# Borda/pyImSegm

Hardware: NVIDIA H100
Metric: megapixels/sec end-to-end SLIC+features+GC (pipe_color2d_slic_features_model_graphcut) (higher is better)
Workload: dtype f64

## Files before the change

### pyimsegm_b200/csrc/graph.cu

```cuda
#include "common.cuh"
#include "block_scan.cuh"
#include <cooperative_groups.h>
namespace cg = cooperative_groups;

namespace {


struct AdjWs {
    unsigned long long* table;
    int* deg;
    int* off;
    int* fill;
    int* tmp_a;
    int* ctr;
    int slots;
};

__device__ __forceinline__ unsigned hash64(unsigned long long k)
{
    k ^= k >> 33; k *= 0xff51afd7ed558ccdull; k ^= k >> 33; k *= 0xc4ceb9fe1a85ec53ull; k ^= k >> 33;
    return (unsigned)k;
}

__device__ void edge_insert(const AdjWs& w, int l0, int l1)
{
    int a = min(l0, l1), b = max(l0, l1);
    unsigned long long key = ((unsigned long long)(unsigned)b << 32) | (unsigned)a;
    unsigned mask = (unsigned)w.slots - 1u;
    unsigned h = hash64(key) & mask;
    for (int probe = 0; probe < w.slots; ++probe) {
        unsigned long long cur = w.table[h];
        if (cur == key) return;
        if (cur == ~0ull) {
            unsigned long long old = atomicCAS(&w.table[h], ~0ull, key);
            if (old == ~0ull) { atomicAdd(&w.deg[b], 1); atomicAdd(&w.ctr[0], 1); return; }
            if (old == key) return;
        }
        h = (h + 1) & mask;
    }
    atomicExch(&w.ctr[1], 1);
}

__global__ void __launch_bounds__(256) k_edge_scan(const int* __restrict__ seg, int H, int W, AdjWs w)
{
    size_t p = (size_t)blockIdx.x * blockDim.x + threadIdx.x;
    if (p >= (size_t)H * W) return;
    int y = (int)(p / W), x = (int)(p % W);
    int l = seg[p];
    if (x + 1 < W) {
        int r = seg[p + 1];
        if (r != l && !(y > 0 && seg[p - W] == l && seg[p - W + 1] == r)) edge_insert(w, l, r);
    }
    if (y + 1 < H) {
        int d = seg[p + W];
        if (d != l && !(x > 0 && seg[p - 1] == l && seg[p + W - 1] == d)) edge_insert(w, l, d);
    }
}

__global__ void __launch_bounds__(256) k_edge_scan3d(const int* __restrict__ seg, int D, int H, int W, AdjWs w)
{
    size_t p = (size_t)blockIdx.x * blockDim.x + threadIdx.x;
    if (p >= (size_t)D * H * W) return;
    const int x = (int)(p % W), y = (int)((p / W) % H), z = (int)(p / ((size_t)H * W));
    const int l = seg[p];
    if (x + 1 < W) { const int r = seg[p + 1]; if (r != l) edge_insert(w, l, r); }
    if (y + 1 < H) { const int d = seg[p + W]; if (d != l) edge_insert(w, l, d); }
    if (z + 1 < D) { const int b = seg[p + (size_t)H * W]; if (b != l) edge_insert(w, l, b); }
}

__global__ void k_centroid3d_acc(const int* __restrict__ seg, int D, int H, int W, unsigned long long* acc)
{
    size_t p = (size_t)blockIdx.x * blockDim.x + threadIdx.x;
    if (p >= (size_t)D * H * W) return;
    const int x = (int)(p % W), y = (int)((p / W) % H), z = (int)(p / ((size_t)H * W));
    unsigned long long* a = acc + 4 * (size_t)seg[p];
    atomicAdd(a, 1ull); atomicAdd(a + 1, (unsigned long long)z); atomicAdd(a + 2, (unsigned long long)y); atomicAdd(a + 3, (unsigned long long)x);
}

__global__ void k_centroid3d_fin(int nb, const unsigned long long* acc, double* centres)
{
    const int k = blockIdx.x * blockDim.x + threadIdx.x;
    if (k >= nb) return;
    const double c = (double)acc[4 * (size_t)k];
    for (int d = 0; d < 3; ++d) centres[3 * (size_t)k + d] = c > 0 ? (double)acc[4 * (size_t)k + 1 + d] / c : -1.0;
}

__global__ void __launch_bounds__(1024) k_edge_offsets(int nb, AdjWs w, int cap, int* n_edges_out)
{
    const int total = cta_scan_chunks<1024, int>(nb, [&](int i) { return w.deg[i]; },
                                                 [&](int i, int off) { w.off[i] = off; w.fill[i] = 0; });
    if (threadIdx.x == 0) {
        w.off[nb] = total;
        *n_edges_out = (w.ctr[1] || total > cap) ? cap + 1 : total;
    }
}

__global__ void k_edge_fill(AdjWs w, int cap)
{
    int i = blockIdx.x * blockDim.x + threadIdx.x;
    if (i >= w.slots) return;
    unsigned long long key = w.table[i];
    if (key == ~0ull) return;
    int b = (int)(key >> 32), a = (int)(key & 0xffffffffu);
    int pos = w.off[b] + atomicAdd(&w.fill[b], 1);
    if (pos < cap) w.tmp_a[pos] = a;
}

__global__ void k_edge_emit(int nb, AdjWs w, int cap, int* __restrict__ edges)
{
    int b = blockIdx.x * blockDim.x + threadIdx.x;
    if (b >= nb) return;
    int beg = w.off[b], end = w.off[b + 1];
    if (end > cap) return;
    for (int i = beg + 1; i < end; ++i) {
        int v = w.tmp_a[i], j = i - 1;
        while (j >= beg && w.tmp_a[j] > v) { w.tmp_a[j + 1] = w.tmp_a[j]; --j; }
        w.tmp_a[j + 1] = v;
    }
    for (int i = beg; i < end; ++i) { edges[2 * (size_t)i] = w.tmp_a[i]; edges[2 * (size_t)i + 1] = b; }
}

static int pow2_at_least(long long v) { int p = 1024; while (p < v) p <<= 1; return p; }

static size_t carve_adj(AdjWs& w, void* ws, size_t bytes, int nb, int cap)
{
    WsCarver c(ws, bytes);
    w.slots = pow2_at_least(2LL * cap);
    w.table = c.take<unsigned long long>((size_t)w.slots);
    w.deg = c.take<int>(nb);
    w.off = c.take<int>((size_t)nb + 1);
    w.fill = c.take<int>(nb);
    w.tmp_a = c.take<int>(cap);
    w.ctr = c.take<int>(4);
    return isb_align(c.off);
}


__device__ double block_sum(double v, double* s_red)
{
#pragma unroll
    for (int o = 16; o > 0; o >>= 1) v += __shfl_xor_sync(0xffffffffu, v, o);
    __syncthreads();
    if ((threadIdx.x & 31) == 0) s_red[threadIdx.x >> 5] = v;
    __syncthreads();
    double t = 0;
    for (int i = 0; i < (int)(blockDim.x >> 5); ++i) t += s_red[i];
    return t;
}

__device__ double block_max(double v, double* s_red)
{
#pragma unroll
    for (int o = 16; o > 0; o >>= 1) v = fmax(v, __shfl_xor_sync(0xffffffffu, v, o));
    __syncthreads();
    if ((threadIdx.x & 31) == 0) s_red[threadIdx.x >> 5] = v;
    __syncthreads();
    double t = s_red[0];
    for (int i = 1; i < (int)(blockDim.x >> 5); ++i) t = fmax(t, s_red[i]);
    return t;
}

constexpr int ECL = 8;

__device__ double cluster_reduce(double v, bool is_max, double* s_red, double* s_x)
{
    const double t = is_max ? block_max(v, s_red) : block_sum(v, s_red);
    cg::cluster_group cl = cg::this_cluster();
    if (threadIdx.x == 0) *s_x = t;
    cl.sync();
    double tot = is_max ? -1.0 : 0.0;
    for (int r = 0; r < ECL; ++r) { const double pr = *cl.map_shared_rank(s_x, r); tot = is_max ? fmax(tot, pr) : tot + pr; }
    cl.sync();
    return tot;
}

__global__ void __cluster_dims__(ECL, 1, 1) __launch_bounds__(1024) k_gc_energies(const double* __restrict__ proba, int N_in, const int* n_nodes_dev, int K, const int* __restrict__ edges, int E_in,
                                                      const int* n_edges_dev, const double* __restrict__ centres,
                                                      const double* __restrict__ vfeat, int D, int metric, int spatial,
                                                      double edge_cost, const double* __restrict__ pairwise, double* unary,
                                                      double* edge_w, int* unary_i, int* edge_wi, int* smooth_i, double* sp)
{
    __shared__ double s_red[32];
    __shared__ double s_x;
    const int tid = blockIdx.x * blockDim.x + threadIdx.x, nth = gridDim.x * blockDim.x;
    const int E = n_edges_dev ? (*n_edges_dev > E_in ? 0 : *n_edges_dev) : E_in;
    const int N = n_nodes_dev ? min(*n_nodes_dev, N_in) : N_in;
    double umax = 0.0;
    for (int i = tid; i < N * K; i += nth) {
        double p = proba[i];
        if (p < 0.01) p = 0.01;
        if (p > 1.0 - 0.01) p = 1.0 - 0.01;
        double u = fabs(-log(p));
        unary[i] = u;
        umax = fmax(umax, fabs(u));
    }
    umax = cluster_reduce(umax, true, s_red, &s_x);
    double dsum = 0.0, ssum = 0.0;
    for (int e = tid; e < E; e += nth) {
        int a = edges[2 * e], b = edges[2 * e + 1];
        double dist = 0.0;
        if (metric != 0) {
            const double* va = vfeat + (size_t)a * D;
            const double* vb = vfeat + (size_t)b * D;
            for (int k = 0; k < D; ++k) {
                double df = va[k] - vb[k];
                if (metric == 1) dist = fmax(dist, df * df);
                else if (metric == 2) dist += fabs(df);
                else dist += df * df;
            }
            if (metric == 3) dist = sqrt(dist);
        }
        edge_w[e] = dist;
        dsum += dist;
        if (spatial) {
            double cy = centres[2 * a] - centres[2 * b], cx = centres[2 * a + 1] - centres[2 * b + 1];
            double s = sqrt(cy * cy + cx * cx);
            sp[e] = s;
            ssum += s;
        }
    }
    dsum = cluster_reduce(dsum, false, s_red, &s_x);
    ssum = cluster_reduce(ssum, false, s_red, &s_x);
    const double dmean = E > 0 ? dsum / E : 0.0, smean = E > 0 ? ssum / E : 1.0;
    double vsum = 0.0;
    if (metric != 0)
        for (int e = tid; e < E; e += nth) { double t = edge_w[e] - dmean; vsum += t * t; }
    vsum = cluster_reduce(vsum, false, s_red, &s_x);
    const double sd = sqrt(E > 0 ? vsum / E : 0.0);
    const double denom = 2.0 * (sd * sd);
    double wmax = 0.0;
    for (int e = tid; e < E; e += nth) {
        double wv = metric != 0 ? exp(-edge_w[e] / denom) : 1.0;
        if (spatial) wv = wv / (sp[e] / smean);
        if (wv < 1e-3) wv = 1e-3;
        if (wv > 1e3) wv = 1e3;
        wv *= edge_cost;
        edge_w[e] = wv;
        wmax = fmax(wmax, fabs(wv));
    }
    wmax = cluster_reduce(wmax, true, s_red, &s_x);
    double pmax = pairwise[0];
    for (int i = 1; i < K * K; ++i) pmax = fmax(pmax, pairwise[i]);
    const double dwf = fmax(umax, wmax * pmax) + 1e-10;
    for (int i = tid; i < N * K; i += nth) unary_i[i] = (int)((unary[i] / dwf) * 100000.0);
    for (int e = tid; e < E; e += nth) { const double wv = edge_w[e]; edge_wi[e] = isnan(wv) ? 0 : (int)((wv / dwf) * 1000.0); }
    for (int i = tid; i < K * K; i += nth) smooth_i[i] = (int)(pairwise[i] * 100.0);
}


__global__ void __launch_bounds__(256) k_gather(const int* __restrict__ seg, long long n, const int* __restrict__ lut_i,
                                                const double* __restrict__ lut_p, int K, int* __restrict__ out_i, double* __restrict__ out_p)
{
    long long p = (long long)blockIdx.x * blockDim.x + threadIdx.x;
    if (p >= n) return;
    int l = seg[p];
    if (out_i) out_i[p] = lut_i[l];
    if (out_p) {
        const double* src = lut_p + (size_t)l * K;
        double* dst = out_p + (size_t)p * K;
        for (int k = 0; k < K; ++k) dst[k] = src[k];
    }
}

}

extern "C" size_t isb_adjacency_workspace_bytes(int nb, int cap)
{
    AdjWs w;
    return carve_adj(w, nullptr, 0, nb, cap);
}

extern "C" int isb_adjacency_edges(const int32_t* seg, int H, int W, int nb, int32_t* edges, int cap, int32_t* n_edges_out, void* ws,
                                   size_t ws_bytes, isb_stream_t stream)
{
    ISB_REQUIRE(seg && edges && n_edges_out && ws, "null pointer");
    ISB_REQUIRE(H > 0 && W > 0 && nb > 0 && cap > 0, "bad sizes");
    AdjWs w;
    size_t need = carve_adj(w, ws, ws_bytes, nb, cap);
    ISB_REQUIRE(need <= ws_bytes, "workspace too small");
    cudaStream_t st = (cudaStream_t)stream;
    ProfScope prof(ISB_PROF_ADJ, st);
    ISB_CUDA_CHECK(cudaMemsetAsync(w.table, 0xFF, sizeof(unsigned long long) * (size_t)w.slots, st));
    ISB_CUDA_CHECK(cudaMemsetAsync(w.deg, 0, sizeof(int) * (size_t)nb, st));
    ISB_CUDA_CHECK(cudaMemsetAsync(w.ctr, 0, sizeof(int) * 4, st));
    size_t n = (size_t)H * W;
    k_edge_scan<<<(unsigned)((n + 255) / 256), 256, 0, st>>>(seg, H, W, w);
    ISB_LAUNCH_CHECK();
    k_edge_offsets<<<1, 1024, 0, st>>>(nb, w, cap, n_edges_out);
    ISB_LAUNCH_CHECK();
    k_edge_fill<<<(w.slots + 255) / 256, 256, 0, st>>>(w, cap);
    ISB_LAUNCH_CHECK();
    k_edge_emit<<<(nb + 127) / 128, 128, 0, st>>>(nb, w, cap, edges);
    ISB_LAUNCH_CHECK();
    return ISB_OK;
}

extern "C" int isb_adjacency_edges_3d(const int32_t* seg, int D, int H, int W, int nb, int32_t* edges, int cap, int32_t* n_edges_out,
                                      void* ws, size_t ws_bytes, isb_stream_t stream)
{
    ISB_REQUIRE(seg && edges && n_edges_out && ws, "null pointer");
    ISB_REQUIRE(D > 0 && H > 0 && W > 0 && nb > 0 && cap > 0, "bad sizes");
    AdjWs w;
    size_t need = carve_adj(w, ws, ws_bytes, nb, cap);
    ISB_REQUIRE(need <= ws_bytes, "workspace too small");
    cudaStream_t st = (cudaStream_t)stream;
    ProfScope prof(ISB_PROF_ADJ, st);
    ISB_CUDA_CHECK(cudaMemsetAsync(w.table, 0xFF, sizeof(unsigned long long) * (size_t)w.slots, st));
    ISB_CUDA_CHECK(cudaMemsetAsync(w.deg, 0, sizeof(int) * (size_t)nb, st));
    ISB_CUDA_CHECK(cudaMemsetAsync(w.ctr, 0, sizeof(int) * 4, st));
    size_t n = (size_t)D * H * W;
    k_edge_scan3d<<<(unsigned)((n + 255) / 256), 256, 0, st>>>(seg, D, H, W, w);
    ISB_LAUNCH_CHECK();
    k_edge_offsets<<<1, 1024, 0, st>>>(nb, w, cap, n_edges_out);
    ISB_LAUNCH_CHECK();
    k_edge_fill<<<(w.slots + 255) / 256, 256, 0, st>>>(w, cap);
    ISB_LAUNCH_CHECK();
    k_edge_emit<<<(nb + 127) / 128, 128, 0, st>>>(nb, w, cap, edges);
    ISB_LAUNCH_CHECK();
    return ISB_OK;
}

extern "C" int isb_centroids_3d(const int32_t* seg, int D, int H, int W, int nb, double* centres, void* ws, size_t ws_bytes, isb_stream_t stream)
{
    ISB_REQUIRE(seg && centres && ws, "null pointer");
    ISB_REQUIRE(D > 0 && H > 0 && W > 0 && nb > 0, "bad sizes");
    ISB_REQUIRE(ws_bytes >= sizeof(unsigned long long) * 4 * (size_t)nb, "workspace too small (4 * nb uint64)");
    cudaStream_t st = (cudaStream_t)stream;
    ISB_CUDA_CHECK(cudaMemsetAsync(ws, 0, sizeof(unsigned long long) * 4 * (size_t)nb, st));
    size_t n = (size_t)D * H * W;
    k_centroid3d_acc<<<(unsigned)((n + 255) / 256), 256, 0, st>>>(seg, D, H, W, (unsigned long long*)ws);
    ISB_LAUNCH_CHECK();
    k_centroid3d_fin<<<(nb + 255) / 256, 256, 0, st>>>(nb, (const unsigned long long*)ws, centres);
    ISB_LAUNCH_CHECK();
    return ISB_OK;
}

extern "C" size_t isb_gc_energies_workspace_bytes(int N, int K, int E) { return isb_align(sizeof(double) * (size_t)(E > 0 ? E : 1)); }

extern "C" int isb_gc_energies(const double* proba, int N, const int32_t* n_nodes_dev, int K, const int32_t* edges, int E, const int32_t* n_edges_dev,
                               const double* centres, int metric, int spatial, double edge_cost, const double* pairwise, double* unary,
                               double* edge_w, int32_t* unary_i, int32_t* edge_wi, int32_t* smooth_i, void* ws, size_t ws_bytes,
                               isb_stream_t stream)
{
    ISB_REQUIRE(proba && edges && pairwise && unary && edge_w && unary_i && edge_wi && smooth_i && ws, "null pointer");
    ISB_REQUIRE(N > 0 && K > 0 && E >= 0, "bad sizes");
    ISB_REQUIRE(metric >= 0 && metric <= 3, "metric must be 0..3");
    ISB_REQUIRE(!spatial || centres, "centres are required for spatially normalised edge weights");
    ISB_REQUIRE(ws_bytes >= isb_gc_energies_workspace_bytes(N, K, E), "workspace too small");
    ProfScope prof(ISB_PROF_ENERGY, (cudaStream_t)stream);
    k_gc_energies<<<ECL, 1024, 0, (cudaStream_t)stream>>>(proba, N, n_nodes_dev, K, edges, E, n_edges_dev, centres, proba, K, metric, spatial, edge_cost,
                                                         pairwise, unary, edge_w, unary_i, edge_wi, smooth_i, (double*)ws);
    ISB_LAUNCH_CHECK();
    return ISB_OK;
}

__global__ void k_fill_i32(int* p, long long n, int v)
{
    long long i = (long long)blockIdx.x * blockDim.x + threadIdx.x;
    if (i < n) p[i] = v;
}

extern "C" int isb_fill_i32(int32_t* dst, long long n, int32_t value, isb_stream_t stream)
{
    ISB_REQUIRE(dst && n > 0, "bad arguments");
    k_fill_i32<<<(unsigned)((n + 255) / 256), 256, 0, (cudaStream_t)stream>>>(dst, n, value);
    ISB_LAUNCH_CHECK();
    return ISB_OK;
}

__global__ void k_combine(void* dst, const void* src, long long n, int op)
{
    long long i = (long long)blockIdx.x * blockDim.x + threadIdx.x;
    if (i >= n) return;
    if (op == 0) ((long long*)dst)[i] += ((const long long*)src)[i];
    else if (op == 1) { long long a = ((long long*)dst)[i], b = ((const long long*)src)[i]; ((long long*)dst)[i] = a > b ? a : b; }
    else if (op == 2) ((double*)dst)[i] = fmin(((double*)dst)[i], ((const double*)src)[i]);
    else if (op == 3) ((double*)dst)[i] = fmax(((double*)dst)[i], ((const double*)src)[i]);
    else ((double*)dst)[i] = ((double*)dst)[i] + ((const double*)src)[i];
}

extern "C" int isb_combine(void* dst, const void* src, long long n, int op, isb_stream_t stream)
{
    ISB_REQUIRE(dst && src && n > 0 && op >= 0 && op <= 4, "bad arguments");
    k_combine<<<(unsigned)((n + 255) / 256), 256, 0, (cudaStream_t)stream>>>(dst, src, n, op);
    ISB_LAUNCH_CHECK();
    return ISB_OK;
}

extern "C" int isb_gather(const int32_t* seg, long long npx, const int32_t* lut_i, const double* lut_p, int K, int32_t* out_i,
                          double* out_p, isb_stream_t stream)
{
    ISB_REQUIRE(seg && npx > 0, "bad arguments");
    ISB_REQUIRE((!out_i || lut_i) && (!out_p || (lut_p && K > 0)), "LUT missing for a requested output");
    ProfScope prof(ISB_PROF_GATHER, (cudaStream_t)stream);
    k_gather<<<(unsigned)((npx + 255) / 256), 256, 0, (cudaStream_t)stream>>>(seg, npx, lut_i, lut_p, K, out_i, out_p);
    ISB_LAUNCH_CHECK();
    return ISB_OK;
}
```

### pyimsegm_b200/csrc/segment_stats.cu

```cuda
#include "common.cuh"

namespace {

constexpr int SROWS = 16;

struct StatWs {
    double* acc;
    double* var;
    long long* iacc;
    float* meanf;
};

__device__ __forceinline__ float clean(float v) { return isnan(v) ? 0.0f : v; }

__global__ void __launch_bounds__(256) k_stats_pass1(const void* __restrict__ img, int dtype, const int* __restrict__ seg, int H, int W,
                                                     int y_off, StatWs ws)
{
    const int x = blockIdx.x * 256 + threadIdx.x;
    if (x >= W) return;
    const int y0 = blockIdx.y * SROWS, y1 = min(y0 + SROWS, H);
    int cur = -1;
    double s0 = 0, s1 = 0, s2 = 0, e0 = 0, e1 = 0, e2 = 0;
    long long cnt = 0, sy = 0;
    for (int y = y0; y <= y1; ++y) {
        int l = -1;
        float v0 = 0, v1 = 0, v2 = 0;
        if (y < y1) {
            size_t p = (size_t)y * W + x;
            l = seg[p];
            if (img) {
                v0 = clean(load_as_f32(img, dtype, 3 * p));
                v1 = clean(load_as_f32(img, dtype, 3 * p + 1));
                v2 = clean(load_as_f32(img, dtype, 3 * p + 2));
            }
        }
        if (l != cur) {
            if (cur >= 0) {
                double* a = ws.acc + 6 * (size_t)cur;
                atomicAdd(a, s0); atomicAdd(a + 1, s1); atomicAdd(a + 2, s2);
                atomicAdd(a + 3, e0); atomicAdd(a + 4, e1); atomicAdd(a + 5, e2);
                unsigned long long* ia = (unsigned long long*)(ws.iacc + 3 * (size_t)cur);
                atomicAdd(ia, (unsigned long long)cnt);
                atomicAdd(ia + 1, (unsigned long long)sy);
                atomicAdd(ia + 2, (unsigned long long)(cnt * x));
            }
            cur = l;
            s0 = s1 = s2 = e0 = e1 = e2 = 0;
            cnt = 0; sy = 0;
        }
        if (y < y1) {
            s0 += (double)v0; s1 += (double)v1; s2 += (double)v2;
            e0 += (double)__fmul_rn(v0, v0); e1 += (double)__fmul_rn(v1, v1); e2 += (double)__fmul_rn(v2, v2);
            cnt += 1; sy += y + y_off;
        }
    }
}

__global__ void k_stats_means(int nb, StatWs ws)
{
    int k = blockIdx.x * blockDim.x + threadIdx.x;
    if (k >= nb) return;
    long long c = ws.iacc[3 * (size_t)k];
    for (int z = 0; z < 3; ++z) {
        double m = ws.acc[6 * (size_t)k + z];
        if (c > 0) m = m / (double)c;
        ws.meanf[3 * (size_t)k + z] = (float)m;
    }
}

__global__ void __launch_bounds__(256) k_stats_pass2(const void* __restrict__ img, int dtype, const int* __restrict__ seg, int H, int W,
                                                     StatWs ws)
{
    const int x = blockIdx.x * 256 + threadIdx.x;
    if (x >= W) return;
    const int y0 = blockIdx.y * SROWS, y1 = min(y0 + SROWS, H);
    int cur = -1;
    double a0 = 0, a1 = 0, a2 = 0;
    float m0 = 0, m1 = 0, m2 = 0;
    for (int y = y0; y <= y1; ++y) {
        int l = -1;
        size_t p = (size_t)y * W + x;
        if (y < y1) l = seg[p];
        if (l != cur) {
            if (cur >= 0) {
                double* a = ws.var + 3 * (size_t)cur;
                atomicAdd(a, a0); atomicAdd(a + 1, a1); atomicAdd(a + 2, a2);
            }
            cur = l;
            a0 = a1 = a2 = 0;
            if (l >= 0) { m0 = ws.meanf[3 * (size_t)l]; m1 = ws.meanf[3 * (size_t)l + 1]; m2 = ws.meanf[3 * (size_t)l + 2]; }
        }
        if (y < y1) {
            float d0 = __fsub_rn(clean(load_as_f32(img, dtype, 3 * p)), m0);
            float d1 = __fsub_rn(clean(load_as_f32(img, dtype, 3 * p + 1)), m1);
            float d2 = __fsub_rn(clean(load_as_f32(img, dtype, 3 * p + 2)), m2);
            a0 += (double)__fmul_rn(d0, d0); a1 += (double)__fmul_rn(d1, d1); a2 += (double)__fmul_rn(d2, d2);
        }
    }
}

__device__ __forceinline__ double tidy(double v)
{
    if (isnan(v)) return 0.0;
    if (isinf(v)) return v > 0 ? 1.7976931348623157e308 : -1.7976931348623157e308;
    return v == 0.0 ? 0.0 : v;
}

__global__ void k_stats_finalize(int nb, int flags, StatWs ws, double* feat, int ld, int col0, double* centres, int* counts)
{
    int k = blockIdx.x * blockDim.x + threadIdx.x;
    if (k >= nb) return;
    long long c = ws.iacc[3 * (size_t)k];
    double dn = (double)c;
    int col = col0;
    double* row = feat ? feat + (size_t)k * ld : nullptr;
    if (row) {
        if (flags & 1) { for (int z = 0; z < 3; ++z) { double v = ws.acc[6 * (size_t)k + z]; if (c > 0) v = v / dn; row[col++] = tidy(v); } }
        if (flags & 2) { for (int z = 0; z < 3; ++z) { double v = ws.var[3 * (size_t)k + z]; if (c > 0) v = v / dn; row[col++] = tidy(sqrt(v)); } }
        if (flags & 4) { for (int z = 0; z < 3; ++z) { double v = ws.acc[6 * (size_t)k + 3 + z]; if (c > 0) v = v / dn; row[col++] = tidy(v); } }
    }
    if (centres) {
        if (c > 0) { centres[2 * (size_t)k] = (double)ws.iacc[3 * (size_t)k + 1] / dn; centres[2 * (size_t)k + 1] = (double)ws.iacc[3 * (size_t)k + 2] / dn; }
        else { centres[2 * (size_t)k] = -1.0; centres[2 * (size_t)k + 1] = -1.0; }
    }
    if (counts) counts[k] = (int)c;
}

static size_t carve(StatWs& w, void* ws, size_t bytes, int nb)
{
    WsCarver c(ws, bytes);
    w.acc = c.take<double>(6 * (size_t)nb);
    w.var = c.take<double>(3 * (size_t)nb);
    w.iacc = c.take<long long>(3 * (size_t)nb);
    w.meanf = c.take<float>(3 * (size_t)nb);
    return isb_align(c.off);
}

}

extern "C" size_t isb_segment_stats_workspace_bytes(int nb)
{
    StatWs w;
    return carve(w, nullptr, 0, nb);
}

extern "C" int isb_segment_stats_2d(const void* img, int dtype, const int32_t* seg, int H, int W, int nb, int flags, double* feat,
                                    int ld, int col0, double* centres, int32_t* counts, void* ws, size_t ws_bytes,
                                    isb_stream_t stream)
{
    ISB_REQUIRE(seg && ws && (img || (flags & 7) == 0), "null pointer");
    ISB_REQUIRE(H > 0 && W > 0 && nb > 0, "bad sizes");
    ISB_REQUIRE(dtype >= ISB_U8 && dtype <= ISB_F64, "bad dtype");
    StatWs w;
    size_t need = carve(w, ws, ws_bytes, nb);
    ISB_REQUIRE(need <= ws_bytes, "workspace too small");
    cudaStream_t st = (cudaStream_t)stream;
    ProfScope prof(ISB_PROF_STATS, st);
    ISB_CUDA_CHECK(cudaMemsetAsync(ws, 0, need, st));
    dim3 grid((W + 255) / 256, (H + SROWS - 1) / SROWS);
    k_stats_pass1<<<grid, 256, 0, st>>>(img, dtype, seg, H, W, 0, w);
    ISB_LAUNCH_CHECK();
    if (flags & 2) {
        k_stats_means<<<(nb + 255) / 256, 256, 0, st>>>(nb, w);
        ISB_LAUNCH_CHECK();
        k_stats_pass2<<<grid, 256, 0, st>>>(img, dtype, seg, H, W, w);
        ISB_LAUNCH_CHECK();
    }
    k_stats_finalize<<<(nb + 255) / 256, 256, 0, st>>>(nb, flags, w, feat, ld, col0, centres, counts);
    ISB_LAUNCH_CHECK();
    return ISB_OK;
}


extern "C" int isb_segment_stats_accumulate(const void* img, int dtype, const int32_t* seg, int H, int W, int y_off, int nb, double* acc,
                                            int64_t* iacc, isb_stream_t stream)
{
    ISB_REQUIRE(seg && acc && iacc, "null pointer");
    ISB_REQUIRE(H > 0 && W > 0 && nb > 0 && y_off >= 0, "bad sizes");
    ISB_REQUIRE(dtype >= ISB_U8 && dtype <= ISB_F64, "bad dtype");
    cudaStream_t st = (cudaStream_t)stream;
    ProfScope prof(ISB_PROF_STATS, st);
    StatWs w;
    w.acc = acc; w.iacc = (long long*)iacc; w.var = nullptr; w.meanf = nullptr;
    dim3 grid((W + 255) / 256, (H + SROWS - 1) / SROWS);
    k_stats_pass1<<<grid, 256, 0, st>>>(img, dtype, seg, H, W, y_off, w);
    ISB_LAUNCH_CHECK();
    return ISB_OK;
}

extern "C" int isb_segment_stats_deviation(const void* img, int dtype, const int32_t* seg, int H, int W, int nb, const double* acc,
                                           const int64_t* iacc, float* meanf_scratch, double* var, isb_stream_t stream)
{
    ISB_REQUIRE(img && seg && acc && iacc && meanf_scratch && var, "null pointer");
    ISB_REQUIRE(H > 0 && W > 0 && nb > 0, "bad sizes");
    ISB_REQUIRE(dtype >= ISB_U8 && dtype <= ISB_F64, "bad dtype");
    cudaStream_t st = (cudaStream_t)stream;
    ProfScope prof(ISB_PROF_STATS, st);
    StatWs w;
    w.acc = (double*)acc; w.iacc = (long long*)iacc; w.var = var; w.meanf = meanf_scratch;
    k_stats_means<<<(nb + 255) / 256, 256, 0, st>>>(nb, w);
    ISB_LAUNCH_CHECK();
    dim3 grid((W + 255) / 256, (H + SROWS - 1) / SROWS);
    k_stats_pass2<<<grid, 256, 0, st>>>(img, dtype, seg, H, W, w);
    ISB_LAUNCH_CHECK();
    return ISB_OK;
}

extern "C" int isb_segment_stats_finish(int nb, int flags, const double* acc, const double* var, const int64_t* iacc, double* feat, int ld,
                                        int col0, double* centres, int32_t* counts, isb_stream_t stream)
{
    ISB_REQUIRE(acc && iacc && (var || !(flags & 2)), "null pointer");
    ISB_REQUIRE(nb > 0, "bad sizes");
    cudaStream_t st = (cudaStream_t)stream;
    StatWs w;
    w.acc = (double*)acc; w.iacc = (long long*)iacc; w.var = (double*)var; w.meanf = nullptr;
    k_stats_finalize<<<(nb + 255) / 256, 256, 0, st>>>(nb, flags, w, feat, ld, col0, centres, counts);
    ISB_LAUNCH_CHECK();
    return ISB_OK;
}
```

Baseline: 1559.

## Dedupe adjacency edges in shared memory, vectorise gather, warp-merge stats atomics

Edge scanning now uses 2D tiles of per-thread row strips, deduplicating edge keys in a per-CTA shared hash set before flushing to the global table. The empty key becomes 0, so a single memset clears the table, degrees and counters. The label gather is vectorised with int4 loads and warp-cooperative double2 stores of probability rows. The stats passes prefetch the next row and merge runs that warp-adjacent lanes share into one atomic per segment via segmented shuffle sums. These changes target global atomic contention and memory traffic, at the cost of more complex code, shared-memory use, and a changed floating-point summation order.

```diff
diff --git a/pyimsegm_b200/csrc/graph.cu b/pyimsegm_b200/csrc/graph.cu
--- a/pyimsegm_b200/csrc/graph.cu
+++ b/pyimsegm_b200/csrc/graph.cu
@@ -8,12 +8,13 @@
 
 struct AdjWs {
     unsigned long long* table;
+    int* ctr;
     int* deg;
     int* off;
     int* fill;
     int* tmp_a;
-    int* ctr;
     int slots;
+    size_t zeroed;
 };
 
 __device__ __forceinline__ unsigned hash64(unsigned long long k)
@@ -22,18 +23,21 @@
     return (unsigned)k;
 }
 
-__device__ void edge_insert(const AdjWs& w, int l0, int l1)
-{
-    int a = min(l0, l1), b = max(l0, l1);
-    unsigned long long key = ((unsigned long long)(unsigned)b << 32) | (unsigned)a;
+__device__ __forceinline__ unsigned long long edge_key(int l0, int l1)
+{
+    return ((unsigned long long)(unsigned)max(l0, l1) << 32) | (unsigned)min(l0, l1);
+}
+
+__device__ void table_insert(const AdjWs& w, unsigned long long key)
+{
     unsigned mask = (unsigned)w.slots - 1u;
     unsigned h = hash64(key) & mask;
     for (int probe = 0; probe < w.slots; ++probe) {
         unsigned long long cur = w.table[h];
         if (cur == key) return;
-        if (cur == ~0ull) {
-            unsigned long long old = atomicCAS(&w.table[h], ~0ull, key);
-            if (old == ~0ull) { atomicAdd(&w.deg[b], 1); atomicAdd(&w.ctr[0], 1); return; }
+        if (cur == 0) {
+            unsigned long long old = atomicCAS(&w.table[h], 0ull, key);
+            if (old == 0) { atomicAdd(&w.deg[key >> 32], 1); atomicAdd(&w.ctr[0], 1); return; }
             if (old == key) return;
         }
         h = (h + 1) & mask;
@@ -41,31 +45,74 @@
     atomicExch(&w.ctr[1], 1);
 }
 
+constexpr int CTA_SLOTS = 512, CTA_PROBES = 32;
+
+__device__ void cta_set_clear(unsigned long long* s)
+{
+    for (int i = threadIdx.x; i < CTA_SLOTS; i += blockDim.x) s[i] = 0;
+    __syncthreads();
+}
+
+__device__ void cta_set_insert(unsigned long long* s, const AdjWs& w, unsigned long long key)
+{
+    unsigned h = hash64(key) & (CTA_SLOTS - 1);
+    for (int probe = 0; probe < CTA_PROBES; ++probe) {
+        unsigned long long cur = s[h];
+        if (cur == key) return;
+        if (cur == 0) {
+            cur = atomicCAS(&s[h], 0ull, key);
+            if (cur == 0 || cur == key) return;
+        }
+        h = (h + 1) & (CTA_SLOTS - 1);
+    }
+    table_insert(w, key);
+}
+
+__device__ void cta_set_flush(const unsigned long long* s, const AdjWs& w)
+{
+    __syncthreads();
+    for (int i = threadIdx.x; i < CTA_SLOTS; i += blockDim.x)
+        if (s[i]) table_insert(w, s[i]);
+}
+
+constexpr int ETW = 64, ETR = 4, ETH = ETR * (256 / ETW);
+
 __global__ void __launch_bounds__(256) k_edge_scan(const int* __restrict__ seg, int H, int W, AdjWs w)
 {
-    size_t p = (size_t)blockIdx.x * blockDim.x + threadIdx.x;
-    if (p >= (size_t)H * W) return;
-    int y = (int)(p / W), x = (int)(p % W);
-    int l = seg[p];
-    if (x + 1 < W) {
-        int r = seg[p + 1];
-        if (r != l && !(y > 0 && seg[p - W] == l && seg[p - W + 1] == r)) edge_insert(w, l, r);
-    }
-    if (y + 1 < H) {
-        int d = seg[p + W];
-        if (d != l && !(x > 0 && seg[p - 1] == l && seg[p + W - 1] == d)) edge_insert(w, l, d);
-    }
+    __shared__ unsigned long long s_set[CTA_SLOTS];
+    cta_set_clear(s_set);
+    const int x = blockIdx.x * ETW + (int)(threadIdx.x % ETW);
+    const int y0 = blockIdx.y * ETH + (int)(threadIdx.x / ETW) * ETR, y1 = min(y0 + ETR, H);
+    if (x < W && y0 < H) {
+        unsigned long long last = 0;
+        int l = seg[(size_t)y0 * W + x];
+        for (int y = y0; y < y1; ++y) {
+            const size_t p = (size_t)y * W + x;
+            const int d = y + 1 < H ? seg[p + W] : l;
+            if (x + 1 < W) {
+                const int r = seg[p + 1];
+                if (r != l && edge_key(l, r) != last) { last = edge_key(l, r); cta_set_insert(s_set, w, last); }
+            }
+            if (d != l && edge_key(l, d) != last) { last = edge_key(l, d); cta_set_insert(s_set, w, last); }
+            l = d;
+        }
+    }
+    cta_set_flush(s_set, w);
 }
 
 __global__ void __launch_bounds__(256) k_edge_scan3d(const int* __restrict__ seg, int D, int H, int W, AdjWs w)
 {
-    size_t p = (size_t)blockIdx.x * blockDim.x + threadIdx.x;
-    if (p >= (size_t)D * H * W) return;
-    const int x = (int)(p % W), y = (int)((p / W) % H), z = (int)(p / ((size_t)H * W));
-    const int l = seg[p];
-    if (x + 1 < W) { const int r = seg[p + 1]; if (r != l) edge_insert(w, l, r); }
-    if (y + 1 < H) { const int d = seg[p + W]; if (d != l) edge_insert(w, l, d); }
-    if (z + 1 < D) { const int b = seg[p + (size_t)H * W]; if (b != l) edge_insert(w, l, b); }
+    __shared__ unsigned long long s_set[CTA_SLOTS];
+    cta_set_clear(s_set);
+    const size_t p = (size_t)blockIdx.x * blockDim.x + threadIdx.x;
+    if (p < (size_t)D * H * W) {
+        const int x = (int)(p % W), y = (int)((p / W) % H), z = (int)(p / ((size_t)H * W));
+        const int l = seg[p];
+        if (x + 1 < W) { const int r = seg[p + 1]; if (r != l) cta_set_insert(s_set, w, edge_key(l, r)); }
+        if (y + 1 < H) { const int d = seg[p + W]; if (d != l) cta_set_insert(s_set, w, edge_key(l, d)); }
+        if (z + 1 < D) { const int b = seg[p + (size_t)H * W]; if (b != l) cta_set_insert(s_set, w, edge_key(l, b)); }
+    }
+    cta_set_flush(s_set, w);
 }
 
 __global__ void k_centroid3d_acc(const int* __restrict__ seg, int D, int H, int W, unsigned long long* acc)
@@ -100,7 +147,7 @@
     int i = blockIdx.x * blockDim.x + threadIdx.x;
     if (i >= w.slots) return;
     unsigned long long key = w.table[i];
-    if (key == ~0ull) return;
+    if (key == 0) return;
     int b = (int)(key >> 32), a = (int)(key & 0xffffffffu);
     int pos = w.off[b] + atomicAdd(&w.fill[b], 1);
     if (pos < cap) w.tmp_a[pos] = a;
@@ -127,11 +174,12 @@
     WsCarver c(ws, bytes);
     w.slots = pow2_at_least(2LL * cap);
     w.table = c.take<unsigned long long>((size_t)w.slots);
+    w.ctr = c.take<int>(4);
     w.deg = c.take<int>(nb);
+    w.zeroed = c.off;
     w.off = c.take<int>((size_t)nb + 1);
     w.fill = c.take<int>(nb);
     w.tmp_a = c.take<int>(cap);
-    w.ctr = c.take<int>(4);
     return isb_align(c.off);
 }
 
@@ -248,17 +296,45 @@
 }
 
 
-__global__ void __launch_bounds__(256) k_gather(const int* __restrict__ seg, long long n, const int* __restrict__ lut_i,
+constexpr int GV = 4, GW = 32 * GV;
+
+__global__ void __launch_bounds__(256) k_gather(const int* __restrict__ seg, long long n, long long n_vec, const int* __restrict__ lut_i,
                                                 const double* __restrict__ lut_p, int K, int* __restrict__ out_i, double* __restrict__ out_p)
 {
-    long long p = (long long)blockIdx.x * blockDim.x + threadIdx.x;
-    if (p >= n) return;
-    int l = seg[p];
-    if (out_i) out_i[p] = lut_i[l];
-    if (out_p) {
-        const double* src = lut_p + (size_t)l * K;
-        double* dst = out_p + (size_t)p * K;
-        for (int k = 0; k < K; ++k) dst[k] = src[k];
+    __shared__ int s_lab[256 * GV];
+    const long long p0 = ((long long)blockIdx.x * blockDim.x + threadIdx.x) * GV;
+    if (p0 >= n) return;
+    if (p0 < n_vec) {
+        const int4 l = *reinterpret_cast<const int4*>(seg + p0);
+        if (out_i) *reinterpret_cast<int4*>(out_i + p0) = make_int4(__ldg(lut_i + l.x), __ldg(lut_i + l.y), __ldg(lut_i + l.z), __ldg(lut_i + l.w));
+        if (out_p) {
+            const int lane = threadIdx.x & 31;
+            *reinterpret_cast<int4*>(s_lab + threadIdx.x * GV) = l;
+            __syncwarp();
+            const int* lab = s_lab + (threadIdx.x - lane) * GV;
+            double2* dst = reinterpret_cast<double2*>(out_p + (p0 - lane * GV) * K);
+            int q = 2 * lane / K, k = 2 * lane % K;
+            const int dq = 64 / K, dk = 64 % K;
+#pragma unroll 2
+            for (int i = lane; i < GW * K / 2; i += 32) {
+                const double v0 = __ldg(lut_p + (size_t)lab[q] * K + k);
+                const int q1 = k + 1 == K ? q + 1 : q, k1 = k + 1 == K ? 0 : k + 1;
+                const double v1 = __ldg(lut_p + (size_t)lab[q1] * K + k1);
+                dst[i] = make_double2(v0, v1);
+                q += dq; k += dk;
+                if (k >= K) { k -= K; ++q; }
+            }
+        }
+        return;
+    }
+    for (long long p = p0; p < min(p0 + GV, n); ++p) {
+        const int l = seg[p];
+        if (out_i) out_i[p] = lut_i[l];
+        if (out_p) {
+            const double* src = lut_p + (size_t)l * K;
+            double* dst = out_p + (size_t)p * K;
+            for (int k = 0; k < K; ++k) dst[k] = src[k];
+        }
     }
 }
 
@@ -275,16 +351,14 @@
 {
     ISB_REQUIRE(seg && edges && n_edges_out && ws, "null pointer");
     ISB_REQUIRE(H > 0 && W > 0 && nb > 0 && cap > 0, "bad sizes");
+    ISB_REQUIRE((H + ETH - 1) / ETH <= 65535, "label map taller than the scan grid (1 048 560 rows)");
     AdjWs w;
     size_t need = carve_adj(w, ws, ws_bytes, nb, cap);
     ISB_REQUIRE(need <= ws_bytes, "workspace too small");
     cudaStream_t st = (cudaStream_t)stream;
     ProfScope prof(ISB_PROF_ADJ, st);
-    ISB_CUDA_CHECK(cudaMemsetAsync(w.table, 0xFF, sizeof(unsigned long long) * (size_t)w.slots, st));
-    ISB_CUDA_CHECK(cudaMemsetAsync(w.deg, 0, sizeof(int) * (size_t)nb, st));
-    ISB_CUDA_CHECK(cudaMemsetAsync(w.ctr, 0, sizeof(int) * 4, st));
-    size_t n = (size_t)H * W;
-    k_edge_scan<<<(unsigned)((n + 255) / 256), 256, 0, st>>>(seg, H, W, w);
+    ISB_CUDA_CHECK(cudaMemsetAsync(w.table, 0, w.zeroed, st));
+    k_edge_scan<<<dim3((W + ETW - 1) / ETW, (H + ETH - 1) / ETH), 256, 0, st>>>(seg, H, W, w);
     ISB_LAUNCH_CHECK();
     k_edge_offsets<<<1, 1024, 0, st>>>(nb, w, cap, n_edges_out);
     ISB_LAUNCH_CHECK();
@@ -305,9 +379,7 @@
     ISB_REQUIRE(need <= ws_bytes, "workspace too small");
     cudaStream_t st = (cudaStream_t)stream;
     ProfScope prof(ISB_PROF_ADJ, st);
-    ISB_CUDA_CHECK(cudaMemsetAsync(w.table, 0xFF, sizeof(unsigned long long) * (size_t)w.slots, st));
-    ISB_CUDA_CHECK(cudaMemsetAsync(w.deg, 0, sizeof(int) * (size_t)nb, st));
-    ISB_CUDA_CHECK(cudaMemsetAsync(w.ctr, 0, sizeof(int) * 4, st));
+    ISB_CUDA_CHECK(cudaMemsetAsync(w.table, 0, w.zeroed, st));
     size_t n = (size_t)D * H * W;
     k_edge_scan3d<<<(unsigned)((n + 255) / 256), 256, 0, st>>>(seg, D, H, W, w);
     ISB_LAUNCH_CHECK();
@@ -393,7 +465,10 @@
     ISB_REQUIRE(seg && npx > 0, "bad arguments");
     ISB_REQUIRE((!out_i || lut_i) && (!out_p || (lut_p && K > 0)), "LUT missing for a requested output");
     ProfScope prof(ISB_PROF_GATHER, (cudaStream_t)stream);
-    k_gather<<<(unsigned)((npx + 255) / 256), 256, 0, (cudaStream_t)stream>>>(seg, npx, lut_i, lut_p, K, out_i, out_p);
-    ISB_LAUNCH_CHECK();
-    return ISB_OK;
-}
+    const bool aligned = (((uintptr_t)seg | (uintptr_t)out_i | (uintptr_t)out_p) & 15) == 0;
+    const long long groups = (npx + GV - 1) / GV;
+    k_gather<<<(unsigned)((groups + 255) / 256), 256, 0, (cudaStream_t)stream>>>(seg, npx, aligned ? npx / GW * GW : 0, lut_i, lut_p, K,
+                                                                                out_i, out_p);
+    ISB_LAUNCH_CHECK();
+    return ISB_OK;
+}
diff --git a/pyimsegm_b200/csrc/segment_stats.cu b/pyimsegm_b200/csrc/segment_stats.cu
--- a/pyimsegm_b200/csrc/segment_stats.cu
+++ b/pyimsegm_b200/csrc/segment_stats.cu
@@ -13,42 +13,76 @@
 
 __device__ __forceinline__ float clean(float v) { return isnan(v) ? 0.0f : v; }
 
+__device__ __forceinline__ int run_segment_end(bool flush, int key, bool* head)
+{
+    const int lane = threadIdx.x & 31;
+    const unsigned fl = __ballot_sync(0xffffffffu, flush);
+    const int prev = __shfl_up_sync(0xffffffffu, key, 1);
+    *head = flush && !(lane > 0 && ((fl >> (lane - 1)) & 1) && prev == key);
+    const unsigned starts = __ballot_sync(0xffffffffu, !flush || *head) & ~((2u << lane) - 1u);
+    return starts ? __ffs(starts) - 1 : 32;
+}
+
+template <typename T> __device__ __forceinline__ T seg_sum(T v, int end)
+{
+    const int lane = threadIdx.x & 31;
+#pragma unroll
+    for (int o = 1; o < 32; o <<= 1) {
+        const T u = __shfl_down_sync(0xffffffffu, v, o);
+        if (lane + o < end) v += u;
+    }
+    return v;
+}
+
 __global__ void __launch_bounds__(256) k_stats_pass1(const void* __restrict__ img, int dtype, const int* __restrict__ seg, int H, int W,
                                                      int y_off, StatWs ws)
 {
     const int x = blockIdx.x * 256 + threadIdx.x;
-    if (x >= W) return;
+    const bool live = x < W;
     const int y0 = blockIdx.y * SROWS, y1 = min(y0 + SROWS, H);
     int cur = -1;
     double s0 = 0, s1 = 0, s2 = 0, e0 = 0, e1 = 0, e2 = 0;
-    long long cnt = 0, sy = 0;
+    int cnt = 0;
+    long long sy = 0;
+    int nl = -1;
+    float n0 = 0, n1 = 0, n2 = 0;
+    auto load = [&](int y) {
+        nl = -1;
+        if (live && y < y1) {
+            const size_t p = (size_t)y * W + x;
+            nl = seg[p];
+            if (img) { n0 = clean(load_as_f32(img, dtype, 3 * p)); n1 = clean(load_as_f32(img, dtype, 3 * p + 1)); n2 = clean(load_as_f32(img, dtype, 3 * p + 2)); }
+        }
+    };
+    load(y0);
     for (int y = y0; y <= y1; ++y) {
-        int l = -1;
-        float v0 = 0, v1 = 0, v2 = 0;
-        if (y < y1) {
-            size_t p = (size_t)y * W + x;
-            l = seg[p];
-            if (img) {
-                v0 = clean(load_as_f32(img, dtype, 3 * p));
-                v1 = clean(load_as_f32(img, dtype, 3 * p + 1));
-                v2 = clean(load_as_f32(img, dtype, 3 * p + 2));
+        const int l = nl;
+        const float v0 = n0, v1 = n1, v2 = n2;
+        load(y + 1);
+        const bool flush = cur >= 0 && l != cur;
+        if (__any_sync(0xffffffffu, flush)) {
+            bool head;
+            const int end = run_segment_end(flush, cur, &head);
+            const double t0 = seg_sum(s0, end), t1 = seg_sum(s1, end), t2 = seg_sum(s2, end);
+            const double u0 = seg_sum(e0, end), u1 = seg_sum(e1, end), u2 = seg_sum(e2, end);
+            const int tc = seg_sum(cnt, end);
+            const long long ty = seg_sum(sy, end), tx = seg_sum((long long)cnt * x, end);
+            if (head) {
+                double* a = ws.acc + 6 * (size_t)cur;
+                atomicAdd(a, t0); atomicAdd(a + 1, t1); atomicAdd(a + 2, t2);
+                atomicAdd(a + 3, u0); atomicAdd(a + 4, u1); atomicAdd(a + 5, u2);
+                unsigned long long* ia = (unsigned long long*)(ws.iacc + 3 * (size_t)cur);
+                atomicAdd(ia, (unsigned long long)tc);
+                atomicAdd(ia + 1, (unsigned long long)ty);
+                atomicAdd(ia + 2, (unsigned long long)tx);
             }
         }
         if (l != cur) {
-            if (cur >= 0) {
-                double* a = ws.acc + 6 * (size_t)cur;
-                atomicAdd(a, s0); atomicAdd(a + 1, s1); atomicAdd(a + 2, s2);
-                atomicAdd(a + 3, e0); atomicAdd(a + 4, e1); atomicAdd(a + 5, e2);
-                unsigned long long* ia = (unsigned long long*)(ws.iacc + 3 * (size_t)cur);
-                atomicAdd(ia, (unsigned long long)cnt);
-                atomicAdd(ia + 1, (unsigned long long)sy);
-                atomicAdd(ia + 2, (unsigned long long)(cnt * x));
-            }
             cur = l;
             s0 = s1 = s2 = e0 = e1 = e2 = 0;
             cnt = 0; sy = 0;
         }
-        if (y < y1) {
+        if (l >= 0) {
             s0 += (double)v0; s1 += (double)v1; s2 += (double)v2;
             e0 += (double)__fmul_rn(v0, v0); e1 += (double)__fmul_rn(v1, v1); e2 += (double)__fmul_rn(v2, v2);
             cnt += 1; sy += y + y_off;
@@ -72,28 +106,43 @@
                                                      StatWs ws)
 {
     const int x = blockIdx.x * 256 + threadIdx.x;
-    if (x >= W) return;
+    const bool live = x < W;
     const int y0 = blockIdx.y * SROWS, y1 = min(y0 + SROWS, H);
     int cur = -1;
     double a0 = 0, a1 = 0, a2 = 0;
     float m0 = 0, m1 = 0, m2 = 0;
+    int nl = -1;
+    float n0 = 0, n1 = 0, n2 = 0;
+    auto load = [&](int y) {
+        nl = -1;
+        if (live && y < y1) {
+            const size_t p = (size_t)y * W + x;
+            nl = seg[p];
+            n0 = clean(load_as_f32(img, dtype, 3 * p)); n1 = clean(load_as_f32(img, dtype, 3 * p + 1)); n2 = clean(load_as_f32(img, dtype, 3 * p + 2));
+        }
+    };
+    load(y0);
     for (int y = y0; y <= y1; ++y) {
-        int l = -1;
-        size_t p = (size_t)y * W + x;
-        if (y < y1) l = seg[p];
+        const int l = nl;
+        const float v0 = n0, v1 = n1, v2 = n2;
+        load(y + 1);
+        const bool flush = cur >= 0 && l != cur;
+        if (__any_sync(0xffffffffu, flush)) {
+            bool head;
+            const int end = run_segment_end(flush, cur, &head);
+            const double t0 = seg_sum(a0, end), t1 = seg_sum(a1, end), t2 = seg_sum(a2, end);
+            if (head) {
+                double* a = ws.var + 3 * (size_t)cur;
+                atomicAdd(a, t0); atomicAdd(a + 1, t1); atomicAdd(a + 2, t2);
+            }
+        }
         if (l != cur) {
-            if (cur >= 0) {
-                double* a = ws.var + 3 * (size_t)cur;
-                atomicAdd(a, a0); atomicAdd(a + 1, a1); atomicAdd(a + 2, a2);
-            }
             cur = l;
             a0 = a1 = a2 = 0;
             if (l >= 0) { m0 = ws.meanf[3 * (size_t)l]; m1 = ws.meanf[3 * (size_t)l + 1]; m2 = ws.meanf[3 * (size_t)l + 2]; }
         }
-        if (y < y1) {
-            float d0 = __fsub_rn(clean(load_as_f32(img, dtype, 3 * p)), m0);
-            float d1 = __fsub_rn(clean(load_as_f32(img, dtype, 3 * p + 1)), m1);
-            float d2 = __fsub_rn(clean(load_as_f32(img, dtype, 3 * p + 2)), m2);
+        if (l >= 0) {
+            const float d0 = __fsub_rn(v0, m0), d1 = __fsub_rn(v1, m1), d2 = __fsub_rn(v2, m2);
             a0 += (double)__fmul_rn(d0, d0); a1 += (double)__fmul_rn(d1, d1); a2 += (double)__fmul_rn(d2, d2);
         }
     }
```

Measured after the change: 1619 (median of 6 runs). +3.9%, better.
